# brianz98/A-Fortran-Electronic-Structure-Program

Measured on AMD Instinct MI355X. Metric: CCSD iter wall-time (s) + (T) wall-time (s); fp64 TFLOP/s vs MFMA peak, higher is better.
Workload: dtype f64; 1 GPU; cfg5: nocc=20 nvirt=200, synthetic hashed ERIs scale 0.005; step = 1 CCSD iteration (replicated) + full (T) over i<=j<=k sharded across ranks; nocc=20, nvirt=200, triples=1540, parallelism=(T) ijk-shard x1, CCSD replicas

## Files before the change

a-fortran-electronic-structure-program_amd/csrc/ccsd.h:

```cpp
#pragma once
#include "afesp_internal.h"

namespace afesp {

struct DiisRing {
    int nerr = 0, nact = 0, it = 0;
    int64_t nvec = 0;
    double *amp = nullptr;
    double *amp_s = nullptr;
    double *hist_t = nullptr, *hist_e = nullptr;
    double *coef = nullptr;
    double *bmat = nullptr;
    bool tail_pending = false;
    int tail_slot = 0, tail_n = 0;
    double tail_b[256];
};
void diis_alloc(Context& cx, DiisRing& r, int diis_nerr);
void diis_save(Context& cx, DiisRing& r);
void diis_update(Context& cx, DiisRing& r);

struct CCState : DiisRing {
    int o = 0, v = 0;
    bool ready = false;
    double* e = nullptr;
// ... 17 lines not shown
    bool r1x_valid = false;
    int hist_plain = 0;
    bool amps_touched = true;
    int64_t pp_nm = 0;
    double *ov_ws = nullptr, *ov_wa = nullptr;
    Tensor I_vo, I_vv, I_oo_p, I_oo, c, asym, x_voov, I_oooo, I_ovov, I_voov, I_ooov_p;
    Tensor z_ooov;
    double energy = 0.0, energy_old = 0.0, rms = 0.0;
    void* tplan = nullptr;
    Tensor I_vovv_pp, I_ooov_pp;
    const double* eri_src = nullptr;
    double* eri_own = nullptr;
    bool have_cr = false;
    int64_t amp_epoch = 0, cr_epoch = 0;
    void* ring = nullptr;
    bool partials_live = false;
    int64_t frozen_id = 0;
};
void triples_plan_free(CCState& s);

bool ring_tg_applies(const CCState& s);
bool ring_tg_pack(Context& cx, CCState& s);
void ring_tg_intermediates(Context& cx, CCState& s);
void ring_tg_residual(Context& cx, CCState& s);
void ring_tg_materialize(Context& cx, CCState& s, const Tensor& I_ovov_out, const Tensor& I_voov_out);
bool ring_live(const CCState& s);
bool ring_res_live(const CCState& s);
void ring_res_clear(CCState& s);
void ring_invalidate(CCState& s);
void ring_reinit(CCState& s);
const double* ring_Y(const CCState& s);
void ring_free(Context& cx, CCState& s);

void ccsd_init(Context& cx, CCState& s, int o, int v, const double* eri_mo_dev, const double* e_host, int diis_nerr);
bool ccsd_can_reinit(const CCState& s, int o, int v, int diis_nerr);
void ccsd_need_vvvv(Context& cx, CCState& s);
void ccsd_refresh_sharding(Context& cx, CCState& s);
bool ccsd_uses_lanes(const CCState& s);
void ccsd_diis_save(Context& cx, CCState& s);
void ccsd_intermediates(Context& cx, CCState& s, bool save_for_diis = false);
void ccsd_amplitudes(Context& cx, CCState& s, bool defer_update = false);
void ccsd_tail_launch(Context& cx, CCState& s);
int ccsd_tail_read(Context& cx, CCState& s, double e_tol, double t_tol);
void ccsd_pp_ladder(Context& cx, CCState& s);
void ccsd_ooov_pair_form(Context& cx, CCState& s, double* out = nullptr, int64_t a0 = 0, int64_t a1 = 0);
const double* ccsd_residual_full(Context& cx, CCState& s, bool r2);
// ... 17 lines not shown
```

a-fortran-electronic-structure-program_amd/csrc/ccsd.hip:

```cpp
#include <algorithm>
#include <cmath>
#include <cstdlib>
#include <cstring>

#include "ccsd.h"
#include "comm.h"
#include "fused.h"

namespace afesp {

static inline int64_t tri64(int64_t i, int64_t j) { return i >= j ? i * (i + 1) / 2 + j : j * (j + 1) / 2 + i; }

bool ccsd_can_reinit(const CCState& s, int o, int v, int diis_nerr)
{
    if (!knobs().cc_reinit) return false;
    return s.ready && s.o == o && s.v == v && s.nerr == diis_nerr && s.pp_sym == pp_sym_pays(o, v);
}

void ccsd_init(Context& cx, CCState& s, int o, int v, const double* eri_mo_dev, const double* e_host, int diis_nerr)
{
    if (o <= 0 || v <= 0) throw Error(1, "ccsd_init: need at least one occupied and one virtual orbital");
    const bool again = ccsd_can_reinit(s, o, v, diis_nerr);
    if (again) {
        cx.quiesce();
        s.ready = false;
        if (s.eri_own) { cx.release(s.eri_own); s.eri_own = nullptr; }
        ring_reinit(s);
        s.cs_packed = s.partials_live = false;
        s.tail_pending = false;
        s.nact = 0; s.it = 0;
        s.hist_plain = 0;
    } else {
        ccsd_free(cx, s);
    }
    s.o = o; s.v = v;
    const int64_t O = o, V = v, n = o + v, ov = O * V, o2v2 = O * O * V * V;
    auto T = [&](Tensor& t, std::initializer_list<int64_t> dims) { if (!again) t = cx.tensor(dims); };
    auto A = [&](double*& ptr, int64_t nd) { if (!again) ptr = cx.alloc(nd); };
    A(s.e, n);
    AFESP_HIP(hipMemcpyAsync(s.e, e_host, sizeof(double) * n, hipMemcpyHostToDevice, cx.stream));
    cx.sync();
    T(s.v_oovv, {O, O, V, V}); T(s.v_ovov, {O, V, O, V}); T(s.v_vvov, {V, V, O, V});
    T(s.v_oovo, {O, O, V, O}); T(s.v_oooo, {O, O, O, O});
// ... 189 lines not shown

void ccsd_intermediates(Context& cx, CCState& s, bool save_for_diis)
{
    auto C = [&](double al, const Tensor& A, const char* la, const Tensor& B, const char* lb, double be, const Tensor& Cc,
                 const char* lc) { contract(cx, al, A, la, B, lb, be, Cc, lc); };
    ccsd_refresh_sharding(cx, s);
    s.amps_touched = false;
    s.r1x_valid = false;
    int64_t v0, v1;
    slice_bounds(s, &v0, &v1);
    auto sl = [&](const Tensor& t, int axis) { return slice_axis(t, axis, v0, v1); };
    if (!(lanes_pay(s) || cx.rec) && ring_tg_applies(s) && ring_tg_pack(cx, s)) {}
    else k_asym_c(cx, s.asym.d, s.c.d, s.t1.d, s.t2.d, s.o, s.v);
    const bool par = lanes_pay(s) && !cx.rec;
    const bool fused = cx.rec != nullptr;
    const bool ring = !par && !fused && ring_tg_applies(s);
    if (!ring) ring_invalidate(s);
    auto lane = [&](int i) { if (par) cx.use_lane(i); };
    if (par) cx.fork(6);
    lane(0);
    C(1.0, s.w_oovv, "miea", s.t1, "me", 0.0, s.I_vo, "ai");
    lane(1);
    const bool ivv_diag = !par && !fused && s.o >= 2;
    if (!ivv_diag) {
        ccsd_need_w_vvov(cx, s);
        C(1.0, s.w_vvov, "ebma", s.t1, "me", 0.0, s.I_vv, "ba");
    }
    if (!s.sharded) C(-1.0, s.w_oovv, "mneb", s.c, "mnea", ivv_diag ? 0.0 : 1.0, s.I_vv, "ba");
    else if (v1 > v0) C(-1.0, s.w_oovv, "mneb", sl(s.c, 3), "mnea", ivv_diag ? 0.0 : 1.0, slice_axis(s.I_vv, 1, v0, v1), "ba");
    lane(0);
    C(1.0, s.w_oovo, "miej", s.t1, "me", 0.0, s.I_oo_p, "ji");
    C(1.0, s.asym, "mjef", s.v_oovv, "mief", 1.0, s.I_oo_p, "ji");
// ... 6 lines not shown
    C(1.0, s.t1, "je", s.I_vo, "ei", 1.0, s.I_oo, "ji");
    lane(1);
    k_copy(cx, s.I_oooo.d, s.v_oooo.d, s.I_oooo.size());
    if (s.pp_sym && !par && !fused) ccsd_oooo_pair_form(cx, s);
    else C(1.0, s.c, "klef", s.v_oovv, "ijef", 1.0, s.I_oooo, "klij");
    C(1.0, s.t1, "ke", s.v_oovo, "ilej", 1.0, s.I_oooo, "klij");
    C(1.0, s.t1, "le", s.v_oovo, "jkei", 1.0, s.I_oooo, "klij");
    lane(2);
    const int64_t a_len = s.I_ovov.stride[3], a_off = v0 * a_len, a_cnt = (v1 - v0) * a_len;
    if (ivv_diag && s.sharded) {
        if (v1 > v0) C(1.0, s.t1, "je", sl(s.v_vvov, 3), "ebia", 0.0, sl(s.I_ovov, 3), "jbia");
    } else if (ivv_diag) {
        contract_pair(cx, {1.0, &s.t1, "je", &s.v_vvov, "ebia", 0.0, &s.I_ovov, "jbia"}, {1.0, &s.v_vvov, "beia", &s.t1, "je", 0.0, &s.x_voov, "bjia"});
    } else if (v1 > v0) {
        k_copy(cx, s.I_ovov.d + a_off, s.v_ovov.d + a_off, a_cnt);
        if (!ring) C(-0.5, s.v_oovv, "mibe", sl(s.c, 2), "mjae", 1.0, sl(s.I_ovov, 3), "jbia");
        C(-1.0, s.v_oovo, "mibj", sl(s.t1, 1), "ma", 1.0, sl(s.I_ovov, 3), "jbia");
        C(1.0, s.t1, "je", sl(s.v_vvov, 3), "ebia", 1.0, sl(s.I_ovov, 3), "jbia");
    }
    lane(3);
    if (s.sharded) { if (v1 > v0) C(1.0, sl(s.v_vvov, 3), "beia", s.t1, "je", 0.0, sl(s.x_voov, 3), "bjia"); }
    else if (!ivv_diag) C(1.0, s.v_vvov, "beia", s.t1, "je", 0.0, s.x_voov, "bjia");
    if (ivv_diag && v1 > v0) {
        k_ivv_diag(cx, s.I_vv.d, s.I_ovov.d, s.x_voov.d, s.o, s.v, (int)v0, (int)v1);
        k_axpby(cx, s.I_ovov.d + a_off, 1.0, s.v_ovov.d + a_off, 1.0, a_cnt);
        if (!ring) C(-0.5, s.v_oovv, "mibe", sl(s.c, 2), "mjae", 1.0, sl(s.I_ovov, 3), "jbia");
        C(-1.0, s.v_oovo, "mibj", sl(s.t1, 1), "ma", 1.0, sl(s.I_ovov, 3), "jbia");
    }
    const int x_voov_ready = par ? cx.mark() : 0;
    if (v1 > v0) {
        permute_add(cx, 1.0, sl(s.v_oovv, 2), "jiab", 0.0, sl(s.I_voov, 3), "bjia");
        if (fused) C(1.0, s.v_vvov, "beia", s.t1, "je", 1.0, s.I_voov, "bjia");
        else k_axpby(cx, s.I_voov.d + a_off, 1.0, s.x_voov.d + a_off, 1.0, a_cnt);
        if (!ring) {
            C(0.5, s.w_oovv, "imbe", sl(s.t2, 3), "mjea", 1.0, sl(s.I_voov, 3), "bjia");
            C(-0.5, s.v_oovv, "imbe", sl(s.c, 2), "mjae", 1.0, sl(s.I_voov, 3), "bjia");
        }
        C(-1.0, s.v_oovo, "imbj", sl(s.t1, 1), "ma", 1.0, sl(s.I_voov, 3), "bjia");
    }
    if (ring) ring_tg_intermediates(cx, s);
    lane(4);
    if (save_for_diis) diis_save(cx, s);
    if (fused) permute_add(cx, 1.0, s.v_oovo, "kjai", 0.0, s.z_ooov, "jkia");
    C(1.0, s.t1, "ie", s.v_oovv, "mjeb", fused ? 1.0 : 0.0, s.z_ooov, "ijmb");
    C(1.0, s.t1, "je", s.v_ovov, "mbie", 1.0, s.z_ooov, "ijmb");
    lane(5);
    permute_add(cx, 1.0, s.v_oovo, "kjai", 0.0, s.I_ooov_p, "jkia");
    if (s.sharded) {
        Tensor osh = view(cx.scratch("ooov_sh", s.I_ooov_p.size()), {(int64_t)s.o, (int64_t)s.o, (int64_t)s.o, (int64_t)s.v});
        if (v1 > v0) {
            if (s.pp_sym) {
                AFESP_HIP(hipMemsetAsync(osh.d + osh.stride[3] * v0, 0, sizeof(double) * osh.stride[3] * (v1 - v0), cx.stream));
                ccsd_ooov_pair_form(cx, s, osh.d, v0, v1);
            } else {
                C(1.0, s.t2, "jkef", sl(s.v_vvov, 3), "efia", 0.0, sl(osh, 3), "jkia");
// ... 159 lines not shown
    if (out == s.I_ooov_p.d && M == O * V && !cx.rec) {
        k_ooov_r1_trace(cx, s.r1x, s.pp_ps, s.ov_wa ? s.pp_pa : nullptr, s.o, s.v, ns, na);
        s.r1x_valid = true;
    }
}

static const char *const R2_LANE2 = "r2_lane2", *const R2_LANE3 = "r2_lane3", *const R1_LANE5 = "r1_lane5";

void ccsd_amplitudes(Context& cx, CCState& s, bool defer_update)
{
    auto C = [&](double al, const Tensor& A, const char* la, const Tensor& B, const char* lb, double be, const Tensor& Cc,
                 const char* lc) { contract(cx, al, A, la, B, lb, be, Cc, lc); };
    ccsd_refresh_sharding(cx, s);
    const bool par = lanes_pay(s) && !cx.rec, sh = s.sharded;
    const bool ring = !par && !cx.rec && !sh && ring_live(s);
    s.partials_live = par;
    ring_res_clear(s);
    int64_t v0, v1;
    slice_bounds(s, &v0, &v1);
    auto sl = [&](const Tensor& t, int axis) { return slice_axis(t, axis, v0, v1); };
    auto lane = [&](int i) { if (par) cx.use_lane(i); };
    Tensor r2b = s.r2, r2c = s.r2, r1b = s.r1;
    Tensor r2s = s.r2;
    if (sh) {
        r2s.d = s.r2_sh;
        const int64_t np = (int64_t)s.v * (s.v + 1) / 2;
        AFESP_HIP(hipMemsetAsync(s.pp, 0, sizeof(double) * ((int64_t)s.o * s.o * np + s.r2.size() + s.r1.size()), cx.stream));
    }
    if (par) {
        r2b.d = cx.scratch(R2_LANE2, s.r2.size());
// ... 18 lines not shown
    lane(1);
    const bool open_with_vvov = !par && !cx.rec && !sh;
    if (ring) ring_tg_residual(cx, s);
    if (open_with_vvov && !s.amps_touched) permute_add(cx, 1.0, s.x_voov, "bija", ring ? 1.0 : 0.0, s.r2, "ijab");
    else if (open_with_vvov) C(1.0, s.t1, "ie", s.v_vvov, "baje", ring ? 1.0 : 0.0, s.r2, "ijab");
    if (!sh) {
        C(1.0, s.t2, "ijae", s.I_vv, "eb", open_with_vvov ? 1.0 : 0.0, s.r2, "ijab");
        C(-1.0, s.t2, "miba", s.I_oo, "jm", 1.0, s.r2, "ijab");
    }
    lane(4);
    ccsd_pp_ladder(cx, s);
    lane(1);
    if (!sh && !(s.pp_sym && !cx.rec)) C(0.5, s.I_oooo, "ijmn", s.c, "mnab", 1.0, s.r2, "ijab");
    lane(2);
    if (ring) {
    } else if (!sh) {
        C(-1.0, s.t2, "mjae", s.I_ovov, "iemb", par ? 0.0 : 1.0, r2b, "ijab");
        C(-1.0, s.I_ovov, "iema", s.t2, "mjeb", 1.0, r2b, "ijab");
    } else if (v1 > v0) {
        C(-1.0, s.t2, "mjae", sl(s.I_ovov, 3), "iemb", 1.0, sl(r2s, 3), "ijab");
        C(-1.0, sl(s.I_ovov, 3), "iema", s.t2, "mjeb", 1.0, sl(r2s, 2), "ijab");
        C(1.0, s.asym, "miea", sl(s.I_voov, 3), "ejmb", 1.0, sl(r2s, 3), "ijab");
        Tensor osh = view(cx.scratch("ooov_sh", s.I_ooov_p.size()), {(int64_t)s.o, (int64_t)s.o, (int64_t)s.o, (int64_t)s.v});
        C(-1.0, s.t1, "ma", sl(osh, 3), "ijmb", 1.0, sl(r2s, 3), "ijab");
        C(1.0, s.t1, "ie", slice_axis(s.v_vvov, 0, v0, v1), "baje", 1.0, sl(r2s, 3), "ijab");
        C(1.0, s.t2, "ijae", slice_axis(s.I_vv, 1, v0, v1), "eb", 1.0, sl(r2s, 3), "ijab");
        C(-1.0, slice_axis(s.t2, 2, v0, v1), "miba", s.I_oo, "jm", 1.0, sl(r2s, 3), "ijab");
        C(0.5, s.I_oooo, "ijmn", sl(s.c, 3), "mnab", 1.0, sl(r2s, 3), "ijab");
        C(-1.0, s.t1, "ma", sl(s.z_ooov, 3), "ijmb", 1.0, sl(r2s, 3), "ijab");
        Tensor r1s = s.r1;
// ... 2 lines not shown
        C(1.0, s.asym, "mief", sl(s.v_vvov, 3), "efma", 1.0, slice_axis(r1s, 1, v0, v1), "ia");
    }
    lane(3);
    if (!sh && !ring) C(1.0, s.asym, "miea", s.I_voov, "ejmb", par ? 0.0 : 1.0, r2c, "ijab");
    if (!open_with_vvov && !sh) C(1.0, s.t1, "ie", s.v_vvov, "baje", 1.0, r2c, "ijab");
    if (!sh) C(-1.0, s.t1, "ma", s.z_ooov, "ijmb", 1.0, r2c, "ijab");
    if (par) cx.join();
    if (sh) {
        const int64_t np = (int64_t)s.v * (s.v + 1) / 2;
        comm_allreduce_dev(cx, cx.comm, s.pp, (int64_t)s.o * s.o * np + s.r2.size() + s.r1.size());
        k_copy(cx, s.r2.d, s.r2_sh, s.r2.size());
        k_axpby(cx, s.r1.d, 1.0, s.r1_sh, 1.0, s.r1.size());
    }
    if (defer_update) return;
    k_t2_update(cx, s.t2.d, s.r2.d, par ? r2b.d : nullptr, par ? r2c.d : nullptr, s.v_oovv.d, s.D2.d, s.pp, s.o, s.v, s.t1.d, s.r1.d,
                par ? r1b.d : nullptr, s.D1.d, ring ? ring_Y(s) : nullptr);
}

const double* ccsd_residual_full(Context& cx, CCState& s, bool r2)
{
    const int64_t n = r2 ? s.r2.size() : s.r1.size();
    double* full = cx.scratch(r2 ? "r2_full" : "r1_full", n);
    auto add_partial = [&](const char* buf) {
        auto it = cx.cache.find(buf);
        if (s.partials_live && it != cx.cache.end()) k_axpby(cx, full, 1.0, (const double*)it->second.first, 1.0, n);
    };
    if (r2) {
        k_r2_full(cx, full, s.r2.d, s.pp, s.o, s.v);
        add_partial(R2_LANE2);
        add_partial(R2_LANE3);
        if (ring_res_live(s)) k_add_swapped(cx, full, ring_Y(s), s.o, s.v);
// ... 213 lines not shown
```

a-fortran-electronic-structure-program_amd/csrc/kernels.hip:

```cpp
#include "device_util.h"
#include "fused.h"

namespace afesp {

namespace {
__global__ void fill_kernel(double* x, int64_t n, double val) { GRID_STRIDE(i, n) x[i] = val; }
__global__ void axpby_kernel(double* y, double a, const double* x, double b, int64_t n)
{
    GRID_STRIDE(i, n) y[i] = a * x[i] + (b != 0.0 ? b * y[i] : 0.0);
}
__global__ void div_kernel(double* out, const double* num, const double* den, int64_t n) { GRID_STRIDE(i, n) out[i] = num[i] / den[i]; }

__global__ void antisym_pair_kernel(double* out, const double* in, int64_t d0, int64_t d1, int64_t d2, int64_t d3, int which)
{
    const int64_t n = d0 * d1 * d2 * d3;
    GRID_STRIDE(x, n)
    {
        int64_t i0 = x % d0, r = x / d0, i1 = r % d1;
        r /= d1;
        int64_t i2 = r % d2, i3 = r / d2;
        int64_t y = which == 0 ? i1 + d0 * (i0 + d1 * (i2 + d2 * i3)) : i0 + d0 * (i1 + d1 * (i3 + d2 * i2));
        out[x] = 2.0 * in[x] - in[y];
    }
}
// ... 15 lines not shown
}

__global__ void t2_update_kernel(double* t2, const double* r2, const double* r2b, const double* r2c, const double* voovv, const double* D2,
                                 const double* pp, int o, int v, double* t1, const double* r1, const double* r1b, const double* D1,
                                 const double* r2y)
{
    const int64_t n = (int64_t)o * o * v * v, n1 = (int64_t)o * v;
    GRID_STRIDE(x, n)
    {
        int i = (int)(x % o);
        int64_t r = x / o;
        int j = (int)(r % o);
        r /= o;
        int a = (int)(r % v), b = (int)(r / v);
        int64_t y = j + (int64_t)o * (i + (int64_t)o * (b + (int64_t)v * a));
        const int64_t lad = (a <= b) ? i + (int64_t)o * (j + (int64_t)o * ((int64_t)b * (b + 1) / 2 + a))
                                     : j + (int64_t)o * (i + (int64_t)o * ((int64_t)a * (a + 1) / 2 + b));
        double rx = r2[x], ry = r2[y];
        if (r2b) { rx += r2b[x]; ry += r2b[y]; }
        if (r2c) { rx += r2c[x]; ry += r2c[y]; }
        if (r2y) {
            rx += r2y[j + (int64_t)o * (i + (int64_t)o * (a + (int64_t)v * b))];
            ry += r2y[i + (int64_t)o * (j + (int64_t)o * (b + (int64_t)v * a))];
        }
        t2[x] = (rx + ry + pp[lad] + voovv[x]) / D2[x];
        if (x < n1) t1[x] = (r1[x] + (r1b ? r1b[x] : 0.0)) / D1[x];
    }
}

__global__ void denominators_kernel(double* D1, double* D2, const double* e, int o, int v)
{
    const int64_t n = (int64_t)o * o * v * v;
    GRID_STRIDE(x, n)
    {
        int i = (int)(x % o);
        int64_t r = x / o;
        int j = (int)(r % o);
        r /= o;
        int a = (int)(r % v), b = (int)(r / v);
        D2[x] = e[i] + e[j] - e[a + o] - e[b + o];
        if (j == 0 && b == 0) D1[i + o * a] = e[i] - e[a + o];
    }
}

__global__ __launch_bounds__(TB) void cc_energy_kernel(double* partial, const double* voovv, const double* t1, const double* t2,
                                                       double* t2_old, int o, int v)
{
    __shared__ double sm[8];
    const int64_t n = (int64_t)o * o * v * v;
    double acc[2] = {0.0, 0.0};
    GRID_STRIDE(x, n)
    {
        int i = (int)(x % o);
        int64_t r = x / o;
        int j = (int)(r % o);
// ... 134 lines not shown
void k_asym_c(Context& cx, double* asym, double* c, const double* t1, const double* t2, int o, int v)
{
    if (cx.rec) {
        const int64_t n2 = (int64_t)o * o * v * v;
        cx.rec->opaque({frange(t1, (int64_t)o * v), frange(t2, n2)}, {frange(asym, n2), frange(c, n2)},
                       [=](Context& c_) { k_asym_c(c_, asym, c, t1, t2, o, v); });
        return;
    }
    LAUNCH(asym_c_kernel, dim3(grid_for((int64_t)o * o * v * v)), asym, c, t1, t2, o, v);
}
__global__ void add_swapped_kernel(double* out, const double* y, int o, int64_t n)
{
    GRID_STRIDE(x, n)
    {
        const int i = (int)(x % o), j = (int)((x / o) % o);
        out[x] += y[x + (int64_t)(j - i) * (1 - o)];
    }
}
void k_add_swapped(Context& cx, double* out, const double* y, int o, int v)
{
    const int64_t n = (int64_t)o * o * v * v;
    LAUNCH(add_swapped_kernel, dim3(grid_for(n)), out, y, o, n);
}
void k_t2_update(Context& cx, double* t2, const double* r2, const double* r2b, const double* r2c, const double* v_oovv, const double* D2,
                 const double* pp, int o, int v, double* t1, const double* r1, const double* r1b, const double* D1, const double* r2y)
{
    if (cx.rec) {
        if (r2y) throw Error(2, "k_t2_update: the exchanged partial residual is not part of a recorded sequence");
        const int64_t n2 = (int64_t)o * o * v * v, n1 = (int64_t)o * v, np = (int64_t)o * o * ((int64_t)v * (v + 1) / 2);
        std::vector<FusedRange> rd = {frange(r2, n2), frange(v_oovv, n2), frange(D2, n2), frange(pp, np), frange(r1, n1), frange(D1, n1)};
        if (r2b) rd.push_back(frange(r2b, n2));
// ... 3 lines not shown
                       [=](Context& c_) { k_t2_update(c_, t2, r2, r2b, r2c, v_oovv, D2, pp, o, v, t1, r1, r1b, D1); });
        return;
    }
    LAUNCH(t2_update_kernel, dim3(grid_for((int64_t)o * o * v * v)), t2, r2, r2b, r2c, v_oovv, D2, pp, o, v, t1, r1, r1b, D1, r2y);
}
__global__ void r2_full_kernel(double* out, const double* r2, const double* pp, int o, int v)
{
    const int64_t n = (int64_t)o * o * v * v;
    GRID_STRIDE(x, n)
    {
        int i = (int)(x % o);
        int64_t r = x / o;
        int j = (int)(r % o);
        r /= o;
        int a = (int)(r % v), b = (int)(r / v);
        const int64_t lad = (a <= b) ? i + (int64_t)o * (j + (int64_t)o * ((int64_t)b * (b + 1) / 2 + a))
                                     : j + (int64_t)o * (i + (int64_t)o * ((int64_t)a * (a + 1) / 2 + b));
        out[x] = r2[x] + 0.5 * pp[lad];
    }
}
void k_r2_full(Context& cx, double* out, const double* r2, const double* pp, int o, int v)
{
    LAUNCH(r2_full_kernel, dim3(grid_for((int64_t)o * o * v * v)), out, r2, pp, o, v);
}
__global__ void vvvv_sympack_packed_kernel(double* vs, double* va, const double* packed, int o, int v, int64_t ks, int64_t ka)
{
    const int64_t V = v, nps = V * (V + 1) / 2, n = V * V * nps;
    GRID_STRIDE(x, n)
    {
        const int e = (int)(x % V), f = (int)((x / V) % V);
        if (e > f) continue;
        const int64_t mp = x / (V * V);
// ... 284 lines not shown
    __shared__ double sm[18 * 4];
    const int o = p.o, v = p.v, ny = p.ny, slot = p.slot;
    const int64_t n = (int64_t)o * o * v * v, n1 = (int64_t)o * v;
    double acc[18];
#pragma unroll
    for (int j = 0; j < 18; ++j) acc[j] = 0.0;
    const int nyc = ny ? ny - 1 : 0;
    GRID_STRIDE(x, n)
    {
        const int i = (int)(x % o);
        int64_t r = x / o;
        const int j = (int)(r % o);
        r /= o;
        const int a = (int)(r % v), b = (int)(r / v);
        const int64_t y = j + (int64_t)o * (i + (int64_t)o * (b + (int64_t)v * a));
        const int64_t lad = (a <= b) ? i + (int64_t)o * (j + (int64_t)o * ((int64_t)b * (b + 1) / 2 + a))
                                     : j + (int64_t)o * (i + (int64_t)o * ((int64_t)a * (a + 1) / 2 + b));
        double r2x = p.r2[x], r2y = p.r2[y];
        const double ppv = p.pp[lad], vx0 = p.voovv[x], d2 = p.D2[x];
        if (YSW) {
            r2x += p.r2y[j + (int64_t)o * (i + (int64_t)o * (a + (int64_t)v * b))];
            r2y += p.r2y[i + (int64_t)o * (j + (int64_t)o * (b + (int64_t)v * a))];
        }
        const double ria = p.r1[i + o * a], dia = p.D1[i + o * a], rjb = p.r1[j + o * b], djb = p.D1[j + o * b];
        const double vx = p.voovv[i + (int64_t)o * (j + (int64_t)o * (b + (int64_t)v * a))];
        const double told = p.t2_old[x];
        double as2 = 0.0, h[NYT > 0 ? NYT : 1];
        const bool half = YSW && p.half;
        const bool hw = !half || a <= b;
        if (NYT > 0) {
            as2 = p.amp_s[n1 + x];
            if (hw) {
#pragma unroll
                for (int q = 0; q < NYT; ++q) h[q] = p.hist_e[(int64_t)min(q, nyc) * p.stride + n1 + x];
            }
        }
        const double t = (r2x + r2y + ppv + vx0) / d2;
// ... 166 lines not shown
```

a-fortran-electronic-structure-program_amd/csrc/ring.hip:

```cpp
#include <algorithm>
#include <cstdlib>
#include <cstring>

#include "ccsd.h"

namespace afesp {

struct RingTg {
    int64_t ov = 0, Kc = 0, each = 0;
    double* slab = nullptr;
    double *cp, *t2p, *t2x, *asp, *nIo, *Ivo, *F1, *F2, *F3, *Y;
    uint32_t* rc32 = nullptr;
    int64_t *cm1 = nullptr, *cn1 = nullptr, *cm2 = nullptr, *cn2 = nullptr;
    int64_t* tab_block = nullptr;
    TgGroup* groups = nullptr;
    int tiles = 0, mx = 0;
    bool pairs2 = false;
    bool frozen_built = false;
    bool packed = false;
    bool live = false;
    bool res_live = false;
};

__global__ __launch_bounds__(256) void ring_tables_kernel(uint32_t* rc32, int64_t* cm1, int64_t* cn1, int64_t* cm2, int64_t* cn2, int o, int v,
                                                          int64_t Kc)
{
// ... 9 lines not shown
            cn2[x] = p + (int64_t)o * o * q;
        }
    }
}

bool ring_tg_applies(const CCState& s)
{
    if (!knobs().ring_tg) return false;
    const int64_t min_ov = knobs().ring_tg_min;
    const int64_t ov = (int64_t)s.o * s.v, Kc = (ov + TG_BK - 1) / TG_BK * TG_BK;
    return !s.sharded && ov >= min_ov && ov >= 2 * TG_BK && 8 * Kc * ov < ((int64_t)1 << 32) - 4096;
}

struct RingPackArgs {
    const double *t1, *t2;
    double *asym, *c, *cp, *t2p, *t2x, *asp;
    int o, v, P, Q;
    int64_t Kc;
    unsigned inv_o, inv_oo;
};
__device__ __forceinline__ unsigned ring_div(unsigned x, unsigned inv) { return inv ? __umulhi(x, inv) : x; }

__global__ __launch_bounds__(256) void ring_pack_kernel(RingPackArgs a)
{
    extern __shared__ double tile[];
    const int o = a.o, v = a.v, oo = o * o, P = a.P, Q = a.Q;
    const int tiles_p = (v + P - 1) / P;
    const int p0 = ((int)blockIdx.x % tiles_p) * P, q0 = ((int)blockIdx.x / tiles_p) * Q;
    const int np = min(P, v - p0), nq = min(Q, v - q0), n = oo * np * nq;
    const unsigned inv_np = np == 1 ? 0u : (unsigned)(((uint64_t)1 << 32) / (unsigned)np + 1);
    const int64_t O = o, V = v;
// ... 9 lines not shown
        const int j = (int)ring_div((unsigned)mj, a.inv_o), m = mj - j * o;
        const int blk = oo * (pp + P * qq);
        const double t = tile[mj + blk], tt = tile[j + o * m + blk];
        const int64_t x = mj + O * O * ((p0 + pp) + V * (q0 + qq));
        a.asym[x] = 2.0 * t - tt;
        a.c[x] = t + a.t1[m + o * (p0 + pp)] * a.t1[j + o * (q0 + qq)];
    }
    for (int idx = threadIdx.x; idx < n; idx += 256) {
        int r = (int)ring_div((unsigned)idx, a.inv_o);
        const int m = idx - r * o;
        int r2 = (int)ring_div((unsigned)r, inv_np);
        const int pp = r - r2 * np;
        const int qq = (int)ring_div((unsigned)r2, a.inv_o), j = r2 - qq * o;
        const int blk = oo * (pp + P * qq);
        const double t = tile[m + o * j + blk], tt = tile[j + o * m + blk];
        const int64_t out = m + O * (p0 + pp) + a.Kc * (j + O * (q0 + qq));
        a.t2p[out] = t;
        a.asp[out] = 2.0 * t - tt;
    }
    const unsigned inv_nq = nq == 1 ? 0u : (unsigned)(((uint64_t)1 << 32) / (unsigned)nq + 1);
    for (int idx = threadIdx.x; idx < n; idx += 256) {
        int r = (int)ring_div((unsigned)idx, a.inv_o);
        const int m = idx - r * o;
        int r2 = (int)ring_div((unsigned)r, inv_nq);
        const int qq = r - r2 * nq;
        const int pp = (int)ring_div((unsigned)r2, a.inv_o), j = r2 - pp * o;
        const double t = tile[m + o * j + oo * (pp + P * qq)];
        const int64_t out = m + O * (q0 + qq) + a.Kc * (j + O * (p0 + pp));
        a.t2x[out] = t;
        a.cp[out] = t + a.t1[m + o * (p0 + pp)] * a.t1[j + o * (q0 + qq)];
    }
}

static RingTg* ring_get(Context& cx, CCState& s)
{
    if (s.ring) return (RingTg*)s.ring;
    RingTg* r = new RingTg();
    s.ring = r;
    const int64_t O = s.o, V = s.v;
    r->ov = O * V;
    r->Kc = (r->ov + TG_BK - 1) / TG_BK * TG_BK;
    r->each = r->Kc * r->ov + 2 * TG_BK;
    r->each = (r->each + 15) / 16 * 16;
    r->slab = cx.alloc(10 * r->each);
    double** bufs[10] = {&r->cp, &r->t2p, &r->t2x, &r->asp, &r->nIo, &r->Ivo, &r->F1, &r->F2, &r->F3, &r->Y};
    for (int q = 0; q < 10; ++q) *bufs[q] = r->slab + q * r->each;
    const int64_t n32 = r->ov + 256, n64 = r->ov + 128;
    int64_t* tab = cx.alloc_i64(4 * n64 + (n32 + 1) / 2 + 8);
    r->cm1 = tab; r->cn1 = tab + n64; r->cm2 = tab + 2 * n64; r->cn2 = tab + 3 * n64;
    r->rc32 = (uint32_t*)(tab + 4 * n64);
    r->tab_block = tab;
    AFESP_KLAUNCH(ring_tables_kernel, dim3((unsigned)std::min<int64_t>((n32 + 255) / 256, 4096)), dim3(256), 0, cx.stream, r->rc32, r->cm1,
                       r->cn1, r->cm2, r->cn2, s.o, s.v, r->Kc);
    AFESP_HIP(hipGetLastError());
    const int M = (int)r->ov, mt = (M + TG_BM - 1) / TG_BM, nt = (M + TG_BN - 1) / TG_BN;
    const int nk1 = (int)(r->Kc / TG_BK), gm = tgemm_group_m(M, nt);
    r->mx = nt;
    r->tiles = 2 * mt * nt;
    auto off = [&](const double* p) { return (int64_t)(p - r->slab); };
    TgGroup g[6] = {};
    auto fill = [&](TgGroup& d, const double* a1, const double* a2, const double* b1, const double* b2, const double* c, const int64_t* cn,
                    int tile0, int nk) {
        d.a1 = off(a1); d.a2 = off(a2); d.b1 = off(b1); d.b2 = off(b2); d.c0 = off(c);
        d.colB = r->rc32; d.offCn = cn;
        d.N = M; d.ntiles = nt; d.tile_start = tile0; d.nk1 = nk1; d.nk = nk;
        d.inv_width = tgemm_inverse(gm * nt);
    };
    fill(g[0], r->t2p, r->cp, r->F2, r->F3, r->Ivo, r->cn1, 0, 2 * nk1);
    fill(g[1], r->cp, r->cp, r->F1, r->F1, r->nIo, r->cn1, mt * nt, nk1);
    g[2].tile_start = 2 * mt * nt;
    fill(g[3], r->t2p, r->Ivo, r->nIo, r->asp, s.r2.d, r->cn2, 0, 2 * nk1);
    fill(g[4], r->nIo, r->nIo, r->t2x, r->t2x, r->Y, r->cn2, mt * nt, nk1);
    g[5].tile_start = 2 * mt * nt;
    r->groups = (TgGroup*)cx.alloc((int64_t)(6 * sizeof(TgGroup) / (sizeof(double)) + 1));
    AFESP_HIP(hipMemcpyAsync(r->groups, g, sizeof(g), hipMemcpyHostToDevice, cx.stream));
    AFESP_HIP(hipStreamSynchronize(cx.stream));
    r->pairs2 = (O % 2 == 0);
    return r;
}

void ring_free(Context& cx, CCState& s)
{
    RingTg* r = (RingTg*)s.ring;
    if (!r) return;
    cx.release(r->slab);
    cx.release(r->tab_block);
    cx.release(r->groups);
    delete r;
    s.ring = nullptr;
}

bool ring_live(const CCState& s) { return s.ring && ((RingTg*)s.ring)->live; }
bool ring_res_live(const CCState& s) { return s.ring && ((RingTg*)s.ring)->res_live; }
void ring_res_clear(CCState& s) { if (s.ring) ((RingTg*)s.ring)->res_live = false; }
const double* ring_Y(const CCState& s) { return ((RingTg*)s.ring)->Y; }

static Tensor kview(const RingTg* r, double* buf, const CCState& s, int pos_m, int pos_p, int pos_x, int pos_e)
{
    Tensor t;
    t.d = buf;
    t.rank = 4;
    const int64_t O = s.o, V = s.v;
    t.dim[pos_m] = O; t.stride[pos_m] = 1;
    t.dim[pos_e] = V; t.stride[pos_e] = O;
    t.dim[pos_p] = O; t.stride[pos_p] = r->Kc;
    t.dim[pos_x] = V; t.stride[pos_x] = r->Kc * O;
    return t;
}

bool ring_tg_pack(Context& cx, CCState& s)
{
    const bool off = !knobs().ring_pack;
    const int64_t oo = (int64_t)s.o * s.o;
    if (off || oo * 8 > 65536 || oo >= 65536 / 4) return false;
    RingTg* r = ring_get(cx, s);
    RingPackArgs a;
    a.t1 = s.t1.d; a.t2 = s.t2.d; a.asym = s.asym.d; a.c = s.c.d;
    a.cp = r->cp; a.t2p = r->t2p; a.t2x = r->t2x; a.asp = r->asp;
    a.o = s.o; a.v = s.v; a.Kc = r->Kc;
    a.P = a.Q = oo * 16 * 8 <= 65536 ? 4 : oo * 4 * 8 <= 65536 ? 2 : 1;
    a.inv_o = tgemm_inverse(s.o);
    a.inv_oo = tgemm_inverse((int)oo);
    const int tiles = ((s.v + a.P - 1) / a.P) * ((s.v + a.Q - 1) / a.Q);
    AFESP_KLAUNCH(ring_pack_kernel, dim3((unsigned)tiles), dim3(256), (size_t)(oo * a.P * a.Q * 8), cx.stream, a);
    AFESP_HIP(hipGetLastError());
    r->packed = true;
    return true;
}

void ring_tg_intermediates(Context& cx, CCState& s)
{
    RingTg* r = ring_get(cx, s);
    if (!r->frozen_built) {
        permute_add(cx, 0.5, s.v_oovv, "mibe", 0.0, kview(r, r->F1, s, 0, 1, 2, 3), "mibe");
        permute_add(cx, 0.5, s.w_oovv, "imbe", 0.0, kview(r, r->F2, s, 1, 0, 2, 3), "imbe");
        permute_add(cx, -0.5, s.v_oovv, "imbe", 0.0, kview(r, r->F3, s, 1, 0, 2, 3), "imbe");
        r->frozen_built = true;
    }
    if (!r->packed) {
        permute_add(cx, 1.0, s.c, "mjae", 0.0, kview(r, r->cp, s, 0, 1, 2, 3), "mjae");
        permute_add(cx, 1.0, s.t2, "mjea", 0.0, kview(r, r->t2p, s, 0, 1, 3, 2), "mjea");
        permute_add(cx, 1.0, s.t2, "mjae", 0.0, kview(r, r->t2x, s, 0, 1, 2, 3), "mjae");
        permute_add(cx, 1.0, s.asym, "miea", 0.0, kview(r, r->asp, s, 0, 1, 3, 2), "miea");
    }
    r->packed = false;
    const int ktail4 = (int)((r->ov - (r->Kc - TG_BK) + 3) / 4);
    TgProblem p{r->slab, r->slab, r->slab, r->rc32, r->cm1, (int)r->ov, true, ktail4};
    p.tag = 1;
    AFESP_HIP(tgemm_launch(p, r->groups, 2, r->tiles, r->mx, cx.stream, cx.tg));
    permute_add(cx, -1.0, s.I_ovov, "jbia", 1.0, kview(r, r->nIo, s, 2, 0, 3, 1), "jbia");
    permute_add(cx, 1.0, s.I_voov, "bjia", 1.0, kview(r, r->Ivo, s, 2, 1, 3, 0), "bjia");
    r->live = true;
}

void ring_tg_residual(Context& cx, CCState& s)
{
    RingTg* r = (RingTg*)s.ring;
    if (!r || !r->live) throw Error(2, "ring_tg_residual: the intermediates of this iteration were not formed on this path");
    const int ktail4 = (int)((r->ov - (r->Kc - TG_BK) + 3) / 4);
    TgProblem p{r->slab, r->slab, r->slab, r->rc32, r->cm2, (int)r->ov, r->pairs2, ktail4};
    p.tag = 1;
    AFESP_HIP(tgemm_launch(p, r->groups + 3, 2, r->tiles, r->mx, cx.stream, cx.tg));
    r->res_live = true;
}

void ring_tg_materialize(Context& cx, CCState& s, const Tensor& I_ovov_out, const Tensor& I_voov_out)
{
    RingTg* r = (RingTg*)s.ring;
    permute_add(cx, -1.0, kview(r, r->nIo, s, 2, 0, 3, 1), "jbia", 0.0, I_ovov_out, "jbia");
    permute_add(cx, 1.0, kview(r, r->Ivo, s, 2, 1, 3, 0), "bjia", 0.0, I_voov_out, "bjia");
}

void ring_reinit(CCState& s)
{
    ring_invalidate(s);
    if (s.ring) ((RingTg*)s.ring)->frozen_built = false;
}

void ring_invalidate(CCState& s)
{
    if (s.ring) { ((RingTg*)s.ring)->live = false; ((RingTg*)s.ring)->res_live = false; ((RingTg*)s.ring)->packed = false; }
}

}
```

a-fortran-electronic-structure-program_amd/csrc/solver.hip:

```cpp
#include <cstdio>
#include <cstring>

#include "solver.h"
#include "integrals.h"

namespace afesp {

void GraphSlot::reset()
{
    if (exec) (void)hipGraphExecDestroy(exec);
    exec = nullptr;
    calls = 0;
    disabled = knobs().no_graph;
}

void Solver::cc_programs_reset(Context& cx)
{
    graph_cc.reset();
    fused_slot_reset(cx, fused_int);
    fused_slot_reset(cx, fused_amp);
    fused_slot_reset(cx, fused_iter);
}

void Solver::destroy(Context& cx)
// ... 191 lines not shown
}

void Solver::get_amplitudes(Context& cx, double* t1, double* t2)
{
    amps_to_host(cx, cc, t1, t2);
    diis_check_flag(cx, host_scalars(cx, DIIS_FLAG_SLOT + 1));
}

void Solver::set_amplitudes(Context& cx, const double* t1, const double* t2)
{
    cc.amp_epoch = ++cx.amp_clock;
    if (ring_live(cc)) {
        ring_tg_materialize(cx, cc, cc.I_ovov, cc.I_voov);
        ring_invalidate(cc);
    }
    cc.amps_touched = true;
    cc.tail_pending = false;
    if (t2) cc.hist_plain = cc.nerr + 1;
    amps_from_host(cx, cc, t1, t2);
}

void Solver::fetch_tensor(Context& cx, const char* name, double* out, int64_t capacity)
{
    CCState& s = cc;
    const int64_t O = s.o, V = s.v;
    struct { const char* n; const Tensor* t; } tab[] = {
        {"v_oovv", &s.v_oovv}, {"v_ovov", &s.v_ovov}, {"v_vvov", &s.v_vvov}, {"v_oovo", &s.v_oovo}, {"v_oooo", &s.v_oooo},
        {"v_vvvv", &s.v_vvvv}, {"I_vo", &s.I_vo}, {"I_vv", &s.I_vv}, {"I_oo_p", &s.I_oo_p}, {"I_oo", &s.I_oo},
        {"c_oovv", &s.c}, {"asym_t2", &s.asym}, {"x_voov", &s.x_voov}, {"I_oooo", &s.I_oooo}, {"I_ovov", &s.I_ovov},
        {"I_voov", &s.I_voov}, {"I_ooov_p", &s.I_ooov_p}, {"r1", &s.r1}, {"r2", &s.r2},
// ... 5 lines not shown
    for (auto& e : tab)
        if (is(e.n)) t = e.t;
    if (!t) throw Error(1, std::string("afesp_ccsd_get_tensor: unknown tensor ") + name);
    if (t->size() > capacity) throw Error(1, std::string("afesp_ccsd_get_tensor: buffer too small for ") + name);
    const double* src = t->d;
    if (t == &vovv) {
        vovv.d = cx.scratch("I_vovv_p", vovv.size());
        ccsd_build_I_vovv_p(cx, s, vovv);
        src = vovv.d;
    } else if (is("r2") || is("r1")) {
        src = ccsd_residual_full(cx, s, is("r2"));
    } else if (ring_live(s) && (is("I_ovov") || is("I_voov"))) {
        Tensor io = view(cx.scratch("ring_I_ovov", t->size()), {O, V, O, V}), iv = view(cx.scratch("ring_I_voov", t->size()), {V, O, O, V});
        ring_tg_materialize(cx, s, io, iv);
        src = is("I_ovov") ? io.d : iv.d;
    }
    AFESP_HIP(hipMemcpyAsync(out, src, sizeof(double) * t->size(), hipMemcpyDeviceToHost, cx.stream));
    cx.sync();
}

double Solver::pp_ladder_flop() const
{
    const double O = cc.o, V = cc.v, ps = V * (V + 1) / 2, pa = V * (V - 1) / 2;
    return cc.pp_sym ? 2.0 * (O * (O + 1) / 2 * ps * ps + O * (O - 1) / 2 * pa * pa) : 2.0 * O * O * V * V * ps;
}

double Solver::iteration_flop() const
{
    const double O = cc.o, V = cc.v, ps = V * (V + 1) / 2, pa = V * (V - 1) / 2, os = O * (O + 1) / 2, oa = O * (O - 1) / 2;
    const bool sym = cc.pp_sym;
    const double pp = pp_ladder_flop();
    const double ooov = sym ? 2.0 * O * V * (os * ps + oa * pa) : 2.0 * O * O * O * V * V * V;
    const double o3v3 = O * O * O * V * V * V;
    const bool large = !ccsd_uses_lanes(cc);
    const double oooo = (sym && large) ? 4.0 * (os * os * ps + oa * oa * pa) : 2.0 * O * O * O * O * V * V;
    const double o2v3 = large ? (sym ? 14.0 : 16.0) : 18.0;
    return pp + ooov + 12.0 * o3v3 + oooo + 2.0 * O * O * O * O * V + o2v3 * O * O * V * V * V + 2.0 * O * V * V * V +
           14.0 * O * O * O * V * V;
}

void Solver::so_init_packed(Context& cx, int nbasis, int nel, const double* host, const double* dev, const double* levels, int diis_nerr,
                            bool foo_as_published)
{
    double* tmp = nullptr;
    if (host) {
        tmp = cx.alloc(neri_of(nbasis));
        AFESP_HIP(hipMemcpyAsync(tmp, host, sizeof(double) * neri_of(nbasis), hipMemcpyHostToDevice, cx.stream));
        dev = tmp;
    }
    cx.drop_scratch("ao2mo_");
    so_programs_reset(cx);
    so_init(cx, so, nbasis, nel, dev, levels, diis_nerr, foo_as_published);
    so.amp_epoch = ++cx.amp_clock;
// ... 96 lines not shown
```

Measured before the change: 60.13 TFLOP/s.

## Reformulate ring terms to cut O3V3 contractions from six to four

Rewrites the CCSD ring intermediates so I_voov absorbs a -1/2 I_ovov permutation and an O3V2 t1 correction, letting the residual use a single t2*I_ovov contraction whose symmetrised half is folded into the amplitude-update kernel. The ring grouped-GEMM path drops the t2p and F3 buffers and halves its K dimension. A new non-ring g_form path does the same with plain contractions, and I_voov is lazily reconstructed when external code needs the conventional form. It also changes the ladder index tie-break for a==b and the D2 summation order, which touches numerics and state-tracking in several places.

```diff
diff --git a/a-fortran-electronic-structure-program_amd/csrc/ccsd.h b/a-fortran-electronic-structure-program_amd/csrc/ccsd.h
--- a/a-fortran-electronic-structure-program_amd/csrc/ccsd.h
+++ b/a-fortran-electronic-structure-program_amd/csrc/ccsd.h
@@ -55,6 +55,8 @@
     bool have_cr = false;
     int64_t amp_epoch = 0, cr_epoch = 0;
     void* ring = nullptr;
+    bool g_form = false, yg_live = false;
+    double* Yg = nullptr;
     bool partials_live = false;
     int64_t frozen_id = 0;
 };
@@ -71,6 +73,7 @@
 void ring_invalidate(CCState& s);
 void ring_reinit(CCState& s);
 const double* ring_Y(const CCState& s);
+void ccsd_I_voov(Context& cx, CCState& s, const Tensor& out);
 void ring_free(Context& cx, CCState& s);
 
 void ccsd_init(Context& cx, CCState& s, int o, int v, const double* eri_mo_dev, const double* e_host, int diis_nerr);
diff --git a/a-fortran-electronic-structure-program_amd/csrc/ccsd.hip b/a-fortran-electronic-structure-program_amd/csrc/ccsd.hip
--- a/a-fortran-electronic-structure-program_amd/csrc/ccsd.hip
+++ b/a-fortran-electronic-structure-program_amd/csrc/ccsd.hip
@@ -26,7 +26,7 @@
         s.ready = false;
         if (s.eri_own) { cx.release(s.eri_own); s.eri_own = nullptr; }
         ring_reinit(s);
-        s.cs_packed = s.partials_live = false;
+        s.cs_packed = s.partials_live = s.g_form = false;
         s.tail_pending = false;
         s.nact = 0; s.it = 0;
         s.hist_plain = 0;
@@ -246,8 +246,10 @@
     else k_asym_c(cx, s.asym.d, s.c.d, s.t1.d, s.t2.d, s.o, s.v);
     const bool par = lanes_pay(s) && !cx.rec;
     const bool fused = cx.rec != nullptr;
-    const bool ring = !par && !fused && ring_tg_applies(s);
+    const bool four = !par && !fused && !s.sharded;
+    const bool ring = four && ring_tg_applies(s);
     if (!ring) ring_invalidate(s);
+    s.g_form = false;
     auto lane = [&](int i) { if (par) cx.use_lane(i); };
     if (par) cx.fork(6);
     lane(0);
@@ -284,7 +286,7 @@
         contract_pair(cx, {1.0, &s.t1, "je", &s.v_vvov, "ebia", 0.0, &s.I_ovov, "jbia"}, {1.0, &s.v_vvov, "beia", &s.t1, "je", 0.0, &s.x_voov, "bjia"});
     } else if (v1 > v0) {
         k_copy(cx, s.I_ovov.d + a_off, s.v_ovov.d + a_off, a_cnt);
-        if (!ring) C(-0.5, s.v_oovv, "mibe", sl(s.c, 2), "mjae", 1.0, sl(s.I_ovov, 3), "jbia");
+        if (!four) C(-0.5, s.v_oovv, "mibe", sl(s.c, 2), "mjae", 1.0, sl(s.I_ovov, 3), "jbia");
         C(-1.0, s.v_oovo, "mibj", sl(s.t1, 1), "ma", 1.0, sl(s.I_ovov, 3), "jbia");
         C(1.0, s.t1, "je", sl(s.v_vvov, 3), "ebia", 1.0, sl(s.I_ovov, 3), "jbia");
     }
@@ -294,7 +296,7 @@
     if (ivv_diag && v1 > v0) {
         k_ivv_diag(cx, s.I_vv.d, s.I_ovov.d, s.x_voov.d, s.o, s.v, (int)v0, (int)v1);
         k_axpby(cx, s.I_ovov.d + a_off, 1.0, s.v_ovov.d + a_off, 1.0, a_cnt);
-        if (!ring) C(-0.5, s.v_oovv, "mibe", sl(s.c, 2), "mjae", 1.0, sl(s.I_ovov, 3), "jbia");
+        if (!four) C(-0.5, s.v_oovv, "mibe", sl(s.c, 2), "mjae", 1.0, sl(s.I_ovov, 3), "jbia");
         C(-1.0, s.v_oovo, "mibj", sl(s.t1, 1), "ma", 1.0, sl(s.I_ovov, 3), "jbia");
     }
     const int x_voov_ready = par ? cx.mark() : 0;
@@ -302,13 +304,28 @@
         permute_add(cx, 1.0, sl(s.v_oovv, 2), "jiab", 0.0, sl(s.I_voov, 3), "bjia");
         if (fused) C(1.0, s.v_vvov, "beia", s.t1, "je", 1.0, s.I_voov, "bjia");
         else k_axpby(cx, s.I_voov.d + a_off, 1.0, s.x_voov.d + a_off, 1.0, a_cnt);
-        if (!ring) {
+        if (!four) {
             C(0.5, s.w_oovv, "imbe", sl(s.t2, 3), "mjea", 1.0, sl(s.I_voov, 3), "bjia");
             C(-0.5, s.v_oovv, "imbe", sl(s.c, 2), "mjae", 1.0, sl(s.I_voov, 3), "bjia");
+            C(-1.0, s.v_oovo, "imbj", sl(s.t1, 1), "ma", 1.0, sl(s.I_voov, 3), "bjia");
         }
-        C(-1.0, s.v_oovo, "imbj", sl(s.t1, 1), "ma", 1.0, sl(s.I_voov, 3), "bjia");
-    }
-    if (ring) ring_tg_intermediates(cx, s);
+    }
+    if (four) {
+        const int64_t O = s.o, V = s.v;
+        Tensor y = view(cx.scratch("ring_y_oovo", s.v_oovo.size()), {O, O, V, O});
+        C(-0.5, s.v_oovv, "imbe", s.t1, "je", 0.0, y, "imbj");
+        C(0.25, s.v_oovv, "mibe", s.t1, "je", 1.0, y, "imbj");
+        k_axpby(cx, y.d, -1.0, s.v_oovo.d, 1.0, y.size());
+        C(1.0, y, "imbj", s.t1, "ma", 1.0, s.I_voov, "bjia");
+        permute_add(cx, -0.5, s.I_ovov, "jbia", 1.0, s.I_voov, "bjia");
+        if (ring) {
+            ring_tg_intermediates(cx, s);
+        } else {
+            C(-0.5, s.v_oovv, "mibe", s.c, "mjae", 1.0, s.I_ovov, "jbia");
+            C(0.25, s.w_oovv, "imbe", s.asym, "mjea", 1.0, s.I_voov, "bjia");
+            s.g_form = true;
+        }
+    }
     lane(4);
     if (save_for_diis) diis_save(cx, s);
     if (fused) permute_add(cx, 1.0, s.v_oovo, "kjai", 0.0, s.z_ooov, "jkia");
@@ -498,6 +515,11 @@
     ccsd_refresh_sharding(cx, s);
     const bool par = lanes_pay(s) && !cx.rec, sh = s.sharded;
     const bool ring = !par && !cx.rec && !sh && ring_live(s);
+    const bool gform = !par && !cx.rec && !sh && !ring && s.g_form;
+    if (s.g_form && !gform) {
+        if (cx.rec) throw Error(2, "ccsd_amplitudes: the intermediates of this iteration were formed outside the recorded sequence");
+        ccsd_I_voov(cx, s, s.I_voov);
+    }
     s.partials_live = par;
     ring_res_clear(s);
     int64_t v0, v1;
@@ -546,6 +568,12 @@
     if (!sh && !(s.pp_sym && !cx.rec)) C(0.5, s.I_oooo, "ijmn", s.c, "mnab", 1.0, s.r2, "ijab");
     lane(2);
     if (ring) {
+    } else if (gform) {
+        s.Yg = cx.scratch("ring_Yg", s.r2.size());
+        Tensor Y = s.r2;
+        Y.d = s.Yg;
+        C(-1.0, s.t2, "mjae", s.I_ovov, "iemb", 0.0, Y, "jiab");
+        s.yg_live = true;
     } else if (!sh) {
         C(-1.0, s.t2, "mjae", s.I_ovov, "iemb", par ? 0.0 : 1.0, r2b, "ijab");
         C(-1.0, s.I_ovov, "iema", s.t2, "mjeb", 1.0, r2b, "ijab");
@@ -578,7 +606,14 @@
     }
     if (defer_update) return;
     k_t2_update(cx, s.t2.d, s.r2.d, par ? r2b.d : nullptr, par ? r2c.d : nullptr, s.v_oovv.d, s.D2.d, s.pp, s.o, s.v, s.t1.d, s.r1.d,
-                par ? r1b.d : nullptr, s.D1.d, ring ? ring_Y(s) : nullptr);
+                par ? r1b.d : nullptr, s.D1.d, ring || gform ? ring_Y(s) : nullptr);
+}
+
+void ccsd_I_voov(Context& cx, CCState& s, const Tensor& out)
+{
+    if (out.d != s.I_voov.d) k_copy(cx, out.d, s.I_voov.d, s.I_voov.size());
+    else s.g_form = false;
+    permute_add(cx, 0.5, s.I_ovov, "jbia", 1.0, out, "bjia");
 }
 
 const double* ccsd_residual_full(Context& cx, CCState& s, bool r2)
diff --git a/a-fortran-electronic-structure-program_amd/csrc/kernels.hip b/a-fortran-electronic-structure-program_amd/csrc/kernels.hip
--- a/a-fortran-electronic-structure-program_amd/csrc/kernels.hip
+++ b/a-fortran-electronic-structure-program_amd/csrc/kernels.hip
@@ -53,14 +53,14 @@
         r /= o;
         int a = (int)(r % v), b = (int)(r / v);
         int64_t y = j + (int64_t)o * (i + (int64_t)o * (b + (int64_t)v * a));
-        const int64_t lad = (a <= b) ? i + (int64_t)o * (j + (int64_t)o * ((int64_t)b * (b + 1) / 2 + a))
-                                     : j + (int64_t)o * (i + (int64_t)o * ((int64_t)a * (a + 1) / 2 + b));
+        const int64_t lad = (a < b || (a == b && i <= j)) ? i + (int64_t)o * (j + (int64_t)o * ((int64_t)b * (b + 1) / 2 + a))
+                                                          : j + (int64_t)o * (i + (int64_t)o * ((int64_t)a * (a + 1) / 2 + b));
         double rx = r2[x], ry = r2[y];
         if (r2b) { rx += r2b[x]; ry += r2b[y]; }
         if (r2c) { rx += r2c[x]; ry += r2c[y]; }
         if (r2y) {
-            rx += r2y[j + (int64_t)o * (i + (int64_t)o * (a + (int64_t)v * b))];
-            ry += r2y[i + (int64_t)o * (j + (int64_t)o * (b + (int64_t)v * a))];
+            rx += fma(0.5, r2y[x], r2y[j + (int64_t)o * (i + (int64_t)o * (a + (int64_t)v * b))]);
+            ry += fma(0.5, r2y[y], r2y[i + (int64_t)o * (j + (int64_t)o * (b + (int64_t)v * a))]);
         }
         t2[x] = (rx + ry + pp[lad] + voovv[x]) / D2[x];
         if (x < n1) t1[x] = (r1[x] + (r1b ? r1b[x] : 0.0)) / D1[x];
@@ -77,7 +77,7 @@
         int j = (int)(r % o);
         r /= o;
         int a = (int)(r % v), b = (int)(r / v);
-        D2[x] = e[i] + e[j] - e[a + o] - e[b + o];
+        D2[x] = (e[i] - e[a + o]) + (e[j] - e[b + o]);
         if (j == 0 && b == 0) D1[i + o * a] = e[i] - e[a + o];
     }
 }
@@ -242,7 +242,7 @@
     GRID_STRIDE(x, n)
     {
         const int i = (int)(x % o), j = (int)((x / o) % o);
-        out[x] += y[x + (int64_t)(j - i) * (1 - o)];
+        out[x] += y[x + (int64_t)(j - i) * (1 - o)] + 0.5 * y[x];
     }
 }
 void k_add_swapped(Context& cx, double* out, const double* y, int o, int v)
@@ -276,8 +276,8 @@
         int j = (int)(r % o);
         r /= o;
         int a = (int)(r % v), b = (int)(r / v);
-        const int64_t lad = (a <= b) ? i + (int64_t)o * (j + (int64_t)o * ((int64_t)b * (b + 1) / 2 + a))
-                                     : j + (int64_t)o * (i + (int64_t)o * ((int64_t)a * (a + 1) / 2 + b));
+        const int64_t lad = (a < b || (a == b && i <= j)) ? i + (int64_t)o * (j + (int64_t)o * ((int64_t)b * (b + 1) / 2 + a))
+                                                          : j + (int64_t)o * (i + (int64_t)o * ((int64_t)a * (a + 1) / 2 + b));
         out[x] = r2[x] + 0.5 * pp[lad];
     }
 }
@@ -592,13 +592,13 @@
         r /= o;
         const int a = (int)(r % v), b = (int)(r / v);
         const int64_t y = j + (int64_t)o * (i + (int64_t)o * (b + (int64_t)v * a));
-        const int64_t lad = (a <= b) ? i + (int64_t)o * (j + (int64_t)o * ((int64_t)b * (b + 1) / 2 + a))
-                                     : j + (int64_t)o * (i + (int64_t)o * ((int64_t)a * (a + 1) / 2 + b));
+        const int64_t lad = (a < b || (a == b && i <= j)) ? i + (int64_t)o * (j + (int64_t)o * ((int64_t)b * (b + 1) / 2 + a))
+                                                          : j + (int64_t)o * (i + (int64_t)o * ((int64_t)a * (a + 1) / 2 + b));
         double r2x = p.r2[x], r2y = p.r2[y];
         const double ppv = p.pp[lad], vx0 = p.voovv[x], d2 = p.D2[x];
         if (YSW) {
-            r2x += p.r2y[j + (int64_t)o * (i + (int64_t)o * (a + (int64_t)v * b))];
-            r2y += p.r2y[i + (int64_t)o * (j + (int64_t)o * (b + (int64_t)v * a))];
+            r2x += fma(0.5, p.r2y[x], p.r2y[j + (int64_t)o * (i + (int64_t)o * (a + (int64_t)v * b))]);
+            r2y += fma(0.5, p.r2y[y], p.r2y[i + (int64_t)o * (j + (int64_t)o * (b + (int64_t)v * a))]);
         }
         const double ria = p.r1[i + o * a], dia = p.D1[i + o * a], rjb = p.r1[j + o * b], djb = p.D1[j + o * b];
         const double vx = p.voovv[i + (int64_t)o * (j + (int64_t)o * (b + (int64_t)v * a))];
diff --git a/a-fortran-electronic-structure-program_amd/csrc/ring.hip b/a-fortran-electronic-structure-program_amd/csrc/ring.hip
--- a/a-fortran-electronic-structure-program_amd/csrc/ring.hip
+++ b/a-fortran-electronic-structure-program_amd/csrc/ring.hip
@@ -9,7 +9,7 @@
 struct RingTg {
     int64_t ov = 0, Kc = 0, each = 0;
     double* slab = nullptr;
-    double *cp, *t2p, *t2x, *asp, *nIo, *Ivo, *F1, *F2, *F3, *Y;
+    double *cp, *t2x, *asp, *nIo, *Ivo, *F1, *F2, *Y;
     uint32_t* rc32 = nullptr;
     int64_t *cm1 = nullptr, *cn1 = nullptr, *cm2 = nullptr, *cn2 = nullptr;
     int64_t* tab_block = nullptr;
@@ -49,7 +49,7 @@
 
 struct RingPackArgs {
     const double *t1, *t2;
-    double *asym, *c, *cp, *t2p, *t2x, *asp;
+    double *asym, *c, *cp, *t2x, *asp;
     int o, v, P, Q;
     int64_t Kc;
     unsigned inv_o, inv_oo;
@@ -89,9 +89,7 @@
         const int qq = (int)ring_div((unsigned)r2, a.inv_o), j = r2 - qq * o;
         const int blk = oo * (pp + P * qq);
         const double t = tile[m + o * j + blk], tt = tile[j + o * m + blk];
-        const int64_t out = m + O * (p0 + pp) + a.Kc * (j + O * (q0 + qq));
-        a.t2p[out] = t;
-        a.asp[out] = 2.0 * t - tt;
+        a.asp[m + O * (p0 + pp) + a.Kc * (j + O * (q0 + qq))] = 2.0 * t - tt;
     }
     const unsigned inv_nq = nq == 1 ? 0u : (unsigned)(((uint64_t)1 << 32) / (unsigned)nq + 1);
     for (int idx = threadIdx.x; idx < n; idx += 256) {
@@ -117,9 +115,9 @@
     r->Kc = (r->ov + TG_BK - 1) / TG_BK * TG_BK;
     r->each = r->Kc * r->ov + 2 * TG_BK;
     r->each = (r->each + 15) / 16 * 16;
-    r->slab = cx.alloc(10 * r->each);
-    double** bufs[10] = {&r->cp, &r->t2p, &r->t2x, &r->asp, &r->nIo, &r->Ivo, &r->F1, &r->F2, &r->F3, &r->Y};
-    for (int q = 0; q < 10; ++q) *bufs[q] = r->slab + q * r->each;
+    r->slab = cx.alloc(8 * r->each);
+    double** bufs[8] = {&r->cp, &r->t2x, &r->asp, &r->nIo, &r->Ivo, &r->F1, &r->F2, &r->Y};
+    for (int q = 0; q < 8; ++q) *bufs[q] = r->slab + q * r->each;
     const int64_t n32 = r->ov + 256, n64 = r->ov + 128;
     int64_t* tab = cx.alloc_i64(4 * n64 + (n32 + 1) / 2 + 8);
     r->cm1 = tab; r->cn1 = tab + n64; r->cm2 = tab + 2 * n64; r->cn2 = tab + 3 * n64;
@@ -134,18 +132,17 @@
     r->tiles = 2 * mt * nt;
     auto off = [&](const double* p) { return (int64_t)(p - r->slab); };
     TgGroup g[6] = {};
-    auto fill = [&](TgGroup& d, const double* a1, const double* a2, const double* b1, const double* b2, const double* c, const int64_t* cn,
-                    int tile0, int nk) {
-        d.a1 = off(a1); d.a2 = off(a2); d.b1 = off(b1); d.b2 = off(b2); d.c0 = off(c);
+    auto fill = [&](TgGroup& d, const double* a, const double* b, const double* c, const int64_t* cn, int tile0) {
+        d.a1 = d.a2 = off(a); d.b1 = d.b2 = off(b); d.c0 = off(c);
         d.colB = r->rc32; d.offCn = cn;
-        d.N = M; d.ntiles = nt; d.tile_start = tile0; d.nk1 = nk1; d.nk = nk;
+        d.N = M; d.ntiles = nt; d.tile_start = tile0; d.nk1 = nk1; d.nk = nk1;
         d.inv_width = tgemm_inverse(gm * nt);
     };
-    fill(g[0], r->t2p, r->cp, r->F2, r->F3, r->Ivo, r->cn1, 0, 2 * nk1);
-    fill(g[1], r->cp, r->cp, r->F1, r->F1, r->nIo, r->cn1, mt * nt, nk1);
+    fill(g[0], r->asp, r->F2, r->Ivo, r->cn1, 0);
+    fill(g[1], r->cp, r->F1, r->nIo, r->cn1, mt * nt);
     g[2].tile_start = 2 * mt * nt;
-    fill(g[3], r->t2p, r->Ivo, r->nIo, r->asp, s.r2.d, r->cn2, 0, 2 * nk1);
-    fill(g[4], r->nIo, r->nIo, r->t2x, r->t2x, r->Y, r->cn2, mt * nt, nk1);
+    fill(g[3], r->Ivo, r->asp, s.r2.d, r->cn2, 0);
+    fill(g[4], r->nIo, r->t2x, r->Y, r->cn2, mt * nt);
     g[5].tile_start = 2 * mt * nt;
     r->groups = (TgGroup*)cx.alloc((int64_t)(6 * sizeof(TgGroup) / (sizeof(double)) + 1));
     AFESP_HIP(hipMemcpyAsync(r->groups, g, sizeof(g), hipMemcpyHostToDevice, cx.stream));
@@ -166,9 +163,9 @@
 }
 
 bool ring_live(const CCState& s) { return s.ring && ((RingTg*)s.ring)->live; }
-bool ring_res_live(const CCState& s) { return s.ring && ((RingTg*)s.ring)->res_live; }
-void ring_res_clear(CCState& s) { if (s.ring) ((RingTg*)s.ring)->res_live = false; }
-const double* ring_Y(const CCState& s) { return ((RingTg*)s.ring)->Y; }
+bool ring_res_live(const CCState& s) { return s.yg_live || (s.ring && ((RingTg*)s.ring)->res_live); }
+void ring_res_clear(CCState& s) { s.yg_live = false; if (s.ring) ((RingTg*)s.ring)->res_live = false; }
+const double* ring_Y(const CCState& s) { return s.yg_live ? s.Yg : ((RingTg*)s.ring)->Y; }
 
 static Tensor kview(const RingTg* r, double* buf, const CCState& s, int pos_m, int pos_p, int pos_x, int pos_e)
 {
@@ -191,7 +188,7 @@
     RingTg* r = ring_get(cx, s);
     RingPackArgs a;
     a.t1 = s.t1.d; a.t2 = s.t2.d; a.asym = s.asym.d; a.c = s.c.d;
-    a.cp = r->cp; a.t2p = r->t2p; a.t2x = r->t2x; a.asp = r->asp;
+    a.cp = r->cp; a.t2x = r->t2x; a.asp = r->asp;
     a.o = s.o; a.v = s.v; a.Kc = r->Kc;
     a.P = a.Q = oo * 16 * 8 <= 65536 ? 4 : oo * 4 * 8 <= 65536 ? 2 : 1;
     a.inv_o = tgemm_inverse(s.o);
@@ -208,13 +205,11 @@
     RingTg* r = ring_get(cx, s);
     if (!r->frozen_built) {
         permute_add(cx, 0.5, s.v_oovv, "mibe", 0.0, kview(r, r->F1, s, 0, 1, 2, 3), "mibe");
-        permute_add(cx, 0.5, s.w_oovv, "imbe", 0.0, kview(r, r->F2, s, 1, 0, 2, 3), "imbe");
-        permute_add(cx, -0.5, s.v_oovv, "imbe", 0.0, kview(r, r->F3, s, 1, 0, 2, 3), "imbe");
+        permute_add(cx, 0.25, s.w_oovv, "imbe", 0.0, kview(r, r->F2, s, 1, 0, 2, 3), "imbe");
         r->frozen_built = true;
     }
     if (!r->packed) {
         permute_add(cx, 1.0, s.c, "mjae", 0.0, kview(r, r->cp, s, 0, 1, 2, 3), "mjae");
-        permute_add(cx, 1.0, s.t2, "mjea", 0.0, kview(r, r->t2p, s, 0, 1, 3, 2), "mjea");
         permute_add(cx, 1.0, s.t2, "mjae", 0.0, kview(r, r->t2x, s, 0, 1, 2, 3), "mjae");
         permute_add(cx, 1.0, s.asym, "miea", 0.0, kview(r, r->asp, s, 0, 1, 3, 2), "miea");
     }
@@ -244,6 +239,7 @@
     RingTg* r = (RingTg*)s.ring;
     permute_add(cx, -1.0, kview(r, r->nIo, s, 2, 0, 3, 1), "jbia", 0.0, I_ovov_out, "jbia");
     permute_add(cx, 1.0, kview(r, r->Ivo, s, 2, 1, 3, 0), "bjia", 0.0, I_voov_out, "bjia");
+    permute_add(cx, -0.5, kview(r, r->nIo, s, 2, 1, 3, 0), "bjia", 1.0, I_voov_out, "bjia");
 }
 
 void ring_reinit(CCState& s)
@@ -254,6 +250,7 @@
 
 void ring_invalidate(CCState& s)
 {
+    s.yg_live = false;
     if (s.ring) { ((RingTg*)s.ring)->live = false; ((RingTg*)s.ring)->res_live = false; ((RingTg*)s.ring)->packed = false; }
 }
 
diff --git a/a-fortran-electronic-structure-program_amd/csrc/solver.hip b/a-fortran-electronic-structure-program_amd/csrc/solver.hip
--- a/a-fortran-electronic-structure-program_amd/csrc/solver.hip
+++ b/a-fortran-electronic-structure-program_amd/csrc/solver.hip
@@ -229,6 +229,7 @@
         ring_tg_materialize(cx, cc, cc.I_ovov, cc.I_voov);
         ring_invalidate(cc);
     }
+    if (cc.g_form) ccsd_I_voov(cx, cc, cc.I_voov);
     cc.amps_touched = true;
     cc.tail_pending = false;
     if (t2) cc.hist_plain = cc.nerr + 1;
@@ -264,6 +265,10 @@
         Tensor io = view(cx.scratch("ring_I_ovov", t->size()), {O, V, O, V}), iv = view(cx.scratch("ring_I_voov", t->size()), {V, O, O, V});
         ring_tg_materialize(cx, s, io, iv);
         src = is("I_ovov") ? io.d : iv.d;
+    } else if (s.g_form && is("I_voov")) {
+        Tensor iv = view(cx.scratch("ring_I_voov", t->size()), {V, O, O, V});
+        ccsd_I_voov(cx, s, iv);
+        src = iv.d;
     }
     AFESP_HIP(hipMemcpyAsync(out, src, sizeof(double) * t->size(), hipMemcpyDeviceToHost, cx.stream));
     cx.sync();
@@ -285,8 +290,9 @@
     const bool large = !ccsd_uses_lanes(cc);
     const double oooo = (sym && large) ? 4.0 * (os * os * ps + oa * oa * pa) : 2.0 * O * O * O * O * V * V;
     const double o2v3 = large ? (sym ? 14.0 : 16.0) : 18.0;
-    return pp + ooov + 12.0 * o3v3 + oooo + 2.0 * O * O * O * O * V + o2v3 * O * O * V * V * V + 2.0 * O * V * V * V +
-           14.0 * O * O * O * V * V;
+    const bool four = large && !cc.sharded;
+    return pp + ooov + (four ? 8.0 : 12.0) * o3v3 + oooo + 2.0 * O * O * O * O * V + o2v3 * O * O * V * V * V + 2.0 * O * V * V * V +
+           (four ? 18.0 : 14.0) * O * O * O * V * V;
 }
 
 void Solver::so_init_packed(Context& cx, int nbasis, int nel, const double* host, const double* dev, const double* levels, int diis_nerr,
```

Result: no change. 59.90 TFLOP/s (-0.4%).
